# mantasu/face-crop-plus

Measured on AMD Instinct MI355X. Metric: faces/sec end-to-end (detect+align+crop), higher is better.
Workload: dtype f16x3; 1 GPU; RetinaFace detect + 5-pt align/crop, batch=32/GPU synthetic 1024x1024 RGB, strategy=largest, det_threshold=0.6, output 256x256, detector on 2 HIP streams x 16 images; global_batch=32, image_size=1024, parallelism=dp1

## Files before the change

face-crop-plus_amd/csrc/fcp_stem_pool.hip:

```cpp
#include "fcp_conv_common.h"

using namespace fcp_conv;

namespace {

typedef _Float16 f16x2 __attribute__((ext_vector_type(2)));

constexpr int PH = 5;
constexpr int SH = 2 * PH + 1;
constexpr int IH = 2 * SH + 5;
constexpr int SPITCH = 68;
constexpr int KSTEPS = 11;

struct StemGeo {
  static constexpr int PW = 16;
  static constexpr int SW = 2 * PW + 1;
  static constexpr int NSTEM = SH * SW;
  static constexpr int NTILES = (NSTEM + 31) / 32;
  static constexpr int IWB = (2 * SW + 5) * 3;
  static constexpr int IPITCH = 6 * SW + 18;
  static constexpr int IN_ELEMS = (IH + 1) * IPITCH;
  static constexpr int NT = 32 * PW;
  static constexpr int NGRP = NT / 128;
  static constexpr int TPR = NT / 28;
  static constexpr int NLOAD = (IWB + TPR - 1) / TPR;
  static constexpr int C1ROWS = (PH * PW + 31) / 32 * 32;
  static constexpr int C1_BYTES = C1ROWS * 2 * 128;
  static constexpr int WGS = 1;
  static_assert(TPR % 3 == 0 && IH * TPR <= NT && IPITCH % 2 == 0 && NTILES % NGRP == 0, "stem patch geometry");
};

struct StemParams {
  const uint8_t* img;
  const float* imgf;
  const uint32_t* wfrag;
  const float* bias;
  const float* wscale;
  float* out;
  int n, h, w, hs, ws, hp, wp, out_ld, out_fmt;
  int tiles_y, tiles_x, npatches;
  int mean[3];
  const char* w1;
  const float* ws1;
  const float* b1;
  float* t1;
  int t1_ld;
};

constexpr int CPITCH = 68;
__device__ __forceinline__ int swz1(int row) { return ((row >> 1) & 7) ^ ((row & 1) << 2); }

__device__ __forceinline__ void lds_barrier() {
  asm volatile("s_waitcnt lgkmcnt(0)" ::: "memory");
  __builtin_amdgcn_s_barrier();
  asm volatile("" ::: "memory");
}

template <bool HAS_C1, bool F32IN = false>
__global__ void __launch_bounds__(StemGeo::NT, StemGeo::WGS) stem_pool_kernel(const StemParams p) {
  static_assert(!(HAS_C1 && F32IN), "the fp32-input stem has no conv1 tail");
  using G = StemGeo;
  constexpr int PW = G::PW, SW = G::SW, NSTEM = G::NSTEM, NTILES = G::NTILES, IWB = G::IWB, IPITCH = G::IPITCH;
  constexpr int IN_ELEMS = G::IN_ELEMS, NT = G::NT, NGRP = G::NGRP, TPR = G::TPR, NLOAD = G::NLOAD, C1ROWS = G::C1ROWS;
  constexpr int KPG = NTILES / NGRP;
  extern __shared__ __attribute__((aligned(16))) float smem[];
  __shared__ __attribute__((aligned(16))) _Float16 inh[IN_ELEMS];
  __shared__ __attribute__((aligned(16))) _Float16 inl[F32IN ? IN_ELEMS : 8];
  float* stage = smem;
  char* c1in = reinterpret_cast<char*>(smem + NSTEM * SPITCH);

  const int tid = threadIdx.x;
  const int lane = tid & 63;
  const int wave = __builtin_amdgcn_readfirstlane(tid >> 6);
  const int half = lane >> 5;

  const int ct = wave & 1, grp = wave >> 1;
  f16x8 wh[KSTEPS], wl[KSTEPS];
#pragma unroll
  for (int q = 0; q < KSTEPS; ++q) {
    const u32x4_t* src = reinterpret_cast<const u32x4_t*>(p.wfrag) + ((ct * KSTEPS + q) * 2) * 64 + lane;
    wh[q] = __builtin_bit_cast(f16x8, src[0]);
    wl[q] = __builtin_bit_cast(f16x8, src[64]);
  }

  const int pc2 = 2 * (tid & 31), pcol = tid >> 5;
  const float ws2a = p.wscale[pc2], ws2b = p.wscale[pc2 + 1], bias2a = p.bias[pc2], bias2b = p.bias[pc2 + 1];
  float ws1a = 0.f, ws1b = 0.f, b1a = 0.f, b1b = 0.f;
  if constexpr (HAS_C1) { ws1a = p.ws1[pc2]; ws1b = p.ws1[pc2 + 1]; b1a = p.b1[pc2]; b1b = p.b1[pc2 + 1]; }
  const int c1rt = wave >> 1, c1ct = wave & 1;

  const int frow = tid / TPR, fc0 = tid - frow * TPR;
  const int fx0 = fc0 / 3, fch = fc0 - fx0 * 3;
  const int fmean = fch == 0 ? p.mean[0] : (fch == 1 ? p.mean[1] : p.mean[2]);
  _Float16* const fdst = inh + min(frow, IH - 1) * IPITCH + fc0;
  uint8_t pre[F32IN ? 1 : NLOAD];
  float pref[F32IN ? NLOAD : 1];
  unsigned pre_ok = 0u;
  auto fetch = [&](int patch) {
    const int pxi = patch % p.tiles_x;
    const int pyi = (patch / p.tiles_x) % p.tiles_y;
    const int ni = patch / (p.tiles_x * p.tiles_y);
    const int iy0 = 4 * pyi * PH - 5, ix0 = 4 * pxi * PW - 5;
    const int y = iy0 + frow;
    const bool rowok = (unsigned)y < (unsigned)p.h && frow < IH;
    const int yc = min(max(y, 0), p.h - 1);
    const uint8_t* base = p.img + ((long)ni * p.h + yc) * p.w * 3 + fch;
    const float* basef = p.imgf + ((long)ni * p.h + yc) * p.w * 4 + fch;
    pre_ok = 0u;
#pragma unroll
    for (int j = 0; j < NLOAD; ++j) {
      const int x = ix0 + fx0 + (TPR / 3) * j;
      pre_ok |= (rowok && (unsigned)x < (unsigned)p.w) ? (1u << j) : 0u;
      if constexpr (F32IN) pref[j] = basef[(unsigned)(min(max(x, 0), p.w - 1) * 4)];
      else pre[j] = base[(unsigned)(min(max(x, 0), p.w - 1) * 3)];
    }
  };
  _Float16* const fdstl = inl + (F32IN ? min(frow, IH - 1) * IPITCH + fc0 : 0);
  auto commit = [&]() {
    if (frow < IH) {
#pragma unroll
      for (int j = 0; j < NLOAD; ++j) {
        if (fc0 + TPR * j < IWB) {
          if constexpr (F32IN) {
            const float v = ((pre_ok >> j) & 1u) ? pref[j] : 0.f;
            const unsigned hu = __builtin_bit_cast(unsigned, __builtin_amdgcn_cvt_pkrtz(v, 0.f));
            const unsigned lu = __builtin_bit_cast(unsigned, __builtin_amdgcn_cvt_pkrtz(fcp_mix_diff<0>(v, hu), 0.f));
            fdst[TPR * j] = __builtin_bit_cast(_Float16, (unsigned short)(hu & 0xFFFFu));
            fdstl[TPR * j] = __builtin_bit_cast(_Float16, (unsigned short)(lu & 0xFFFFu));
          } else {
            fdst[TPR * j] = (_Float16)(float)(((pre_ok >> j) & 1u) ? (int)pre[j] - fmean : 0);
          }
        }
      }
    }
  };

  for (int i = tid; i < IN_ELEMS / 2; i += NT) {
    reinterpret_cast<uint32_t*>(inh)[i] = 0u;
    if constexpr (F32IN) reinterpret_cast<uint32_t*>(inl)[i] = 0u;
  }
  __syncthreads();

  int abase_t[KPG];
#pragma unroll
  for (int k = 0; k < KPG; ++k) {
    int pix = (grp + NGRP * k) * 32 + (lane & 31);
    pix = pix < NSTEM ? pix : NSTEM - 1;
    const int si = pix / SW, sj = pix - si * SW;
    abase_t[k] = (2 * si) * IPITCH + 6 * sj;
  }

  int patch = blockIdx.x;
  if (patch < p.npatches) fetch(patch);
  for (; patch < p.npatches; patch += gridDim.x) {
    commit();
    lds_barrier();
    const int next = patch + gridDim.x;
    if (next < p.npatches) fetch(next);

    const int pxi = patch % p.tiles_x;
    const int pyi = (patch / p.tiles_x) % p.tiles_y;
    const int ni = patch / (p.tiles_x * p.tiles_y);
    const int py0 = pyi * PH, px0 = pxi * PW;
    const int sy0 = 2 * py0 - 1, sx0 = 2 * px0 - 1;
    const bool interior = sy0 >= 0 && sy0 + SH <= p.hs && sx0 >= 0 && sx0 + SW <= p.ws;

#pragma unroll
    for (int k = 0; k < KPG; ++k) {
      const int t = grp + NGRP * k;
      const int abase = abase_t[k];
      f32x16 acc;
#pragma unroll
      for (int e = 0; e < 16; ++e) acc[e] = 0.f;
      auto afrag_of = [&](const _Float16* plane, int q) {
        const int ch = 2 * q + half;
        const int kh = ch / 3, part = ch - kh * 3;
        const uint32_t* wp = reinterpret_cast<const uint32_t*>(plane + abase + kh * IPITCH + 8 * part);
        const u32x4_t raw = {wp[0], wp[1], wp[2], wp[3]};
        return __builtin_bit_cast(f16x8, raw);
      };
      auto afrag = [&](int q) { return afrag_of(inh, q); };
      f16x8 a = afrag(0), al = a;
      if constexpr (F32IN) al = afrag_of(inl, 0);
#pragma unroll
      for (int q = 0; q < KSTEPS; ++q) {
        f16x8 an = a, aln = al;
        if (q + 1 < KSTEPS) {
          an = afrag(q + 1);
          if constexpr (F32IN) aln = afrag_of(inl, q + 1);
        }
        __builtin_amdgcn_sched_barrier(0);
        if constexpr (F32IN) {
          acc = __builtin_amdgcn_mfma_f32_32x32x16_f16(wh[q], al, acc, 0, 0, 0);
          acc = __builtin_amdgcn_mfma_f32_32x32x16_f16(wl[q], a, acc, 0, 0, 0);
          acc = __builtin_amdgcn_mfma_f32_32x32x16_f16(wh[q], a, acc, 0, 0, 0);
        } else {
          acc = __builtin_amdgcn_mfma_f32_32x32x16_f16(wl[q], a, acc, 0, 0, 0);
          acc = __builtin_amdgcn_mfma_f32_32x32x16_f16(wh[q], a, acc, 0, 0, 0);
        }
        a = an; al = aln;
      }
      {
        const int row = t * 32 + (lane & 31);
        bool in = true;
        if (!interior) {
          const int si = row / SW, sj = row - si * SW;
          in = (unsigned)(sy0 + si) < (unsigned)p.hs && (unsigned)(sx0 + sj) < (unsigned)p.ws;
        }
        if (row < NSTEM) {
          float* dst = stage + row * SPITCH + ct * 32 + 4 * half;
#pragma unroll
          for (int g = 0; g < 4; ++g)
            *reinterpret_cast<f32x4*>(dst + 8 * g) = in ? f32x4{acc[4 * g], acc[4 * g + 1], acc[4 * g + 2], acc[4 * g + 3]}
                                                        : f32x4{-INFINITY, -INFINITY, -INFINITY, -INFINITY};
        }
      }
    }
    lds_barrier();

    f16x8 c1w[8];
    if constexpr (HAS_C1) {
      if (c1rt < C1ROWS / 32) {
        const char* wrow = p.w1 + (size_t)(c1ct * 32 + (lane & 31)) * 256;
#pragma unroll
        for (int sl = 0; sl < 2; ++sl)
#pragma unroll
          for (int sh = 0; sh < 2; ++sh) {
            c1w[(sl * 2 + sh) * 2] = *reinterpret_cast<const f16x8*>(wrow + sl * 128 + (2 * sh + half) * 16);
            c1w[(sl * 2 + sh) * 2 + 1] = *reinterpret_cast<const f16x8*>(wrow + sl * 128 + (4 + 2 * sh + half) * 16);
          }
      }
    }
    {
      typedef float f32x2 __attribute__((ext_vector_type(2)));
      const float* sp = stage + (2 * pcol) * SPITCH + pc2;
      f32x2 rm[SH];
#pragma unroll
      for (int si = 0; si < SH; ++si) {
        const f32x2 a = *reinterpret_cast<const f32x2*>(sp + (si * SW) * SPITCH);
        const f32x2 b = *reinterpret_cast<const f32x2*>(sp + (si * SW + 1) * SPITCH);
        const f32x2 c = *reinterpret_cast<const f32x2*>(sp + (si * SW + 2) * SPITCH);
        rm[si][0] = fmaxf(fmaxf(a[0], b[0]), c[0]);
        rm[si][1] = fmaxf(fmaxf(a[1], b[1]), c[1]);
      }
      const int ox = px0 + pcol;
#pragma unroll
      for (int py = 0; py < PH; ++py) {
        const int oy = py0 + py;
        if (oy >= p.hp || ox >= p.wp) continue;
        float v0 = fmaxf(fmaxf(rm[2 * py][0], rm[2 * py + 1][0]), rm[2 * py + 2][0]) * ws2a + bias2a;
        float v1 = fmaxf(fmaxf(rm[2 * py][1], rm[2 * py + 1][1]), rm[2 * py + 2][1]) * ws2b + bias2b;
        v0 = v0 > 0.f ? v0 : 0.f;
        v1 = v1 > 0.f ? v1 : 0.f;
        const long pixel = ((long)ni * p.hp + oy) * p.wp + ox;
        if (p.out_fmt == 1) {
          unsigned hu, lu;
          split2(v0, v1, hu, lu);
          char* ob = reinterpret_cast<char*>(p.out) + pixel * p.out_ld * 4 + split_chan_off(pc2);
          *reinterpret_cast<unsigned*>(ob) = hu;
          *reinterpret_cast<unsigned*>(ob + 64) = lu;
          if constexpr (HAS_C1) {
            const int pp = py * PW + pcol;
            const int q = (pc2 & 31) >> 3, sw = swz1(pp);
            char* trow = c1in + pp * 256 + (pc2 >> 5) * 128 + (pc2 & 7) * 2;
            *reinterpret_cast<unsigned*>(trow + ((q ^ sw) << 4)) = hu;
            *reinterpret_cast<unsigned*>(trow + (((4 + q) ^ sw) << 4)) = lu;
          }
        } else {
          *reinterpret_cast<f32x2*>(p.out + pixel * p.out_ld + pc2) = f32x2{v0, v1};
        }
      }
    }
    if constexpr (HAS_C1) {
      lds_barrier();
      if (c1rt < C1ROWS / 32) {
        f32x16 acc;
#pragma unroll
        for (int e = 0; e < 16; ++e) acc[e] = 0.f;
        const int row = c1rt * 32 + (lane & 31), sw = swz1(row);
        const char* arow = c1in + row * 256;
#pragma unroll
        for (int sl = 0; sl < 2; ++sl)
#pragma unroll
          for (int sh = 0; sh < 2; ++sh) {
            const f16x8 bh = c1w[(sl * 2 + sh) * 2], bl = c1w[(sl * 2 + sh) * 2 + 1];
            const f16x8 ah = *reinterpret_cast<const f16x8*>(arow + sl * 128 + (((2 * sh + half) ^ sw) << 4));
            const f16x8 al = *reinterpret_cast<const f16x8*>(arow + sl * 128 + (((4 + 2 * sh + half) ^ sw) << 4));
            acc = __builtin_amdgcn_mfma_f32_32x32x16_f16(bh, al, acc, 0, 0, 0);
            acc = __builtin_amdgcn_mfma_f32_32x32x16_f16(bl, ah, acc, 0, 0, 0);
            acc = __builtin_amdgcn_mfma_f32_32x32x16_f16(bh, ah, acc, 0, 0, 0);
          }
        float* dst = stage + row * CPITCH + c1ct * 32 + 4 * half;
#pragma unroll
        for (int g = 0; g < 4; ++g)
          *reinterpret_cast<f32x4*>(dst + 8 * g) = f32x4{acc[4 * g], acc[4 * g + 1], acc[4 * g + 2], acc[4 * g + 3]};
      }
      lds_barrier();
      {
        typedef float f32x2 __attribute__((ext_vector_type(2)));
        const int ox = px0 + pcol;
        f32x2 cv[PH];
#pragma unroll
        for (int py = 0; py < PH; ++py) cv[py] = *reinterpret_cast<const f32x2*>(stage + (py * PW + pcol) * CPITCH + pc2);
#pragma unroll
        for (int py = 0; py < PH; ++py) {
          const int oy = py0 + py;
          if (oy >= p.hp || ox >= p.wp) continue;
          const float x0 = conv_value_relu(cv[py][0], ws1a, b1a), x1 = conv_value_relu(cv[py][1], ws1b, b1b);
          unsigned hu, lu;
          split2(x0, x1, hu, lu);
          const long pixel = ((long)ni * p.hp + oy) * p.wp + ox;
          char* ob = reinterpret_cast<char*>(p.t1) + pixel * p.t1_ld * 4 + split_chan_off(pc2);
          *reinterpret_cast<unsigned*>(ob) = hu;
          *reinterpret_cast<unsigned*>(ob + 64) = lu;
        }
      }
    }
    lds_barrier();
  }
}

}

extern "C" int fcp_stem7x7s2_relu_pool_conv1_u8(const uint8_t* images, int n, int h, int w, const int32_t* mean_rgb,
                                                const void* wfrag, const float* bias, const float* wscale, float* out,
                                                int out_ld, int out_fmt, const void* w1, const float* ws1, const float* b1,
                                                float* t1, int t1_ld, fcp_stream_t stream) {
  FCP_REQUIRE(images && wfrag && bias && wscale && out && mean_rgb, "stem: null pointer");
  const bool has_c1 = w1 != nullptr;
  if (has_c1) {
    FCP_REQUIRE(ws1 && b1 && t1, "stem + conv1: conv1 needs its scales, bias and output");
    FCP_REQUIRE(out_fmt == 1, "stem + conv1: the pooled map must be written in split32 (its bytes are conv1's operand)");
    FCP_REQUIRE(t1_ld >= 64 && t1_ld % 32 == 0 && ((uintptr_t)t1 & 127) == 0 && ((uintptr_t)w1 & 15) == 0,
                "stem + conv1: misaligned conv1 filter / output view");
  }
  FCP_REQUIRE(n > 0 && h >= 1 && w >= 1 && (long)h * w * 3 < (1L << 31), "stem: bad image size");
  FCP_REQUIRE((unsigned)out_fmt <= 1u, "stem: out_fmt must be 0 (fp32) or 1 (split32)");
  FCP_REQUIRE(out_ld >= 64 && out_ld % (out_fmt ? 32 : 4) == 0 && ((uintptr_t)out & (out_fmt ? 127 : 15)) == 0,
              "stem: misaligned output view");
  FCP_REQUIRE(((uintptr_t)wfrag & 15) == 0, "stem: filter fragments must be 16-byte aligned");
  for (int c = 0; c < 3; ++c) FCP_REQUIRE(mean_rgb[c] >= 0 && mean_rgb[c] <= 255, "stem: means must be integers in 0..255");
  StemParams p = {};
  p.img = images; p.wfrag = static_cast<const uint32_t*>(wfrag); p.bias = bias; p.wscale = wscale; p.out = out;
  p.n = n; p.h = h; p.w = w;
  p.hs = (h + 6 - 7) / 2 + 1; p.ws = (w + 6 - 7) / 2 + 1;
  p.hp = (p.hs + 2 - 3) / 2 + 1; p.wp = (p.ws + 2 - 3) / 2 + 1;
  p.out_ld = out_ld; p.out_fmt = out_fmt;
  p.tiles_y = fcp_cdiv(p.hp, PH); p.tiles_x = fcp_cdiv(p.wp, StemGeo::PW);
  const long np = (long)n * p.tiles_y * p.tiles_x;
  FCP_REQUIRE(np < (1L << 31) && (long)n * h * w * 3 < (1L << 40), "stem: batch too large");
  p.npatches = (int)np;
  for (int c = 0; c < 3; ++c) p.mean[c] = mean_rgb[c];
  p.w1 = static_cast<const char*>(w1); p.ws1 = ws1; p.b1 = b1; p.t1 = t1; p.t1_ld = t1_ld;
  using G = StemGeo;
  const size_t lds = (size_t)G::NSTEM * SPITCH * 4 + (has_c1 ? G::C1_BYTES : 0);
  const int cus = fcp_cu_count() * G::WGS;
  const int grid = (int)(np < cus ? np : cus);
  if (has_c1) {
    FCP_LDS_OPT_IN((&stem_pool_kernel<true>), lds);
    hipLaunchKernelGGL((stem_pool_kernel<true>), dim3(grid), dim3(G::NT), lds, (hipStream_t)stream, p);
  } else {
    FCP_LDS_OPT_IN((&stem_pool_kernel<false>), lds);
    hipLaunchKernelGGL((stem_pool_kernel<false>), dim3(grid), dim3(G::NT), lds, (hipStream_t)stream, p);
  }
  FCP_LAUNCH_OK();
  return 0;
}

extern "C" int fcp_stem7x7s2_relu_pool_f32(const float* x4, int n, int h, int w, const void* wfrag, const float* bias,
                                           const float* wscale, float* out, int out_ld, int out_fmt, fcp_stream_t stream) {
  FCP_REQUIRE(x4 && wfrag && bias && wscale && out, "stem(f32): null pointer");
  FCP_REQUIRE(n > 0 && h >= 1 && w >= 1 && (long)h * w * 4 < (1L << 31), "stem(f32): bad image size");
  FCP_REQUIRE((unsigned)out_fmt <= 1u, "stem(f32): out_fmt must be 0 (fp32) or 1 (split32)");
  FCP_REQUIRE(out_ld >= 64 && out_ld % (out_fmt ? 32 : 4) == 0 && ((uintptr_t)out & (out_fmt ? 127 : 15)) == 0,
              "stem(f32): misaligned output view");
  FCP_REQUIRE(((uintptr_t)wfrag & 15) == 0 && ((uintptr_t)x4 & 15) == 0, "stem(f32): input / filter fragments must be 16-byte aligned");
  using G = StemGeo;
  StemParams p = {};
  p.imgf = x4; p.wfrag = static_cast<const uint32_t*>(wfrag); p.bias = bias; p.wscale = wscale; p.out = out;
  p.n = n; p.h = h; p.w = w;
  p.hs = (h + 6 - 7) / 2 + 1; p.ws = (w + 6 - 7) / 2 + 1;
  p.hp = (p.hs + 2 - 3) / 2 + 1; p.wp = (p.ws + 2 - 3) / 2 + 1;
  p.out_ld = out_ld; p.out_fmt = out_fmt;
  p.tiles_y = fcp_cdiv(p.hp, PH); p.tiles_x = fcp_cdiv(p.wp, G::PW);
  const long np = (long)n * p.tiles_y * p.tiles_x;
  FCP_REQUIRE(np < (1L << 31) && (long)n * h * w * 4 < (1L << 40), "stem(f32): batch too large");
  p.npatches = (int)np;
  const size_t lds = (size_t)G::NSTEM * SPITCH * 4;
  const int cus = fcp_cu_count() * G::WGS;
  const int grid = (int)(np < cus ? np : cus);
  FCP_LDS_OPT_IN((&stem_pool_kernel<false, true>), lds);
  hipLaunchKernelGGL((stem_pool_kernel<false, true>), dim3(grid), dim3(G::NT), lds, (hipStream_t)stream, p);
  FCP_LAUNCH_OK();
  return 0;
}

extern "C" int fcp_stem7x7s2_relu_pool_u8(const uint8_t* images, int n, int h, int w, const int32_t* mean_rgb,
                                          const void* wfrag, const float* bias, const float* wscale, float* out,
                                          int out_ld, int out_fmt, fcp_stream_t stream) {
  return fcp_stem7x7s2_relu_pool_conv1_u8(images, n, h, w, mean_rgb, wfrag, bias, wscale, out, out_ld, out_fmt, nullptr, nullptr,
                                          nullptr, nullptr, 0, stream);
}
```

Before: 1457 faces/s.

## Warp-specialize stem kernel into MFMA and load/pool waves with double-buffered input

Splits the stem workgroup into matrix waves, which run the 7x7 conv MFMAs and the conv1 tail, and service waves, which fetch the next patch into a double-buffered LDS input tile and do the 3x3 max-pool plus output. The stem tiles are computed in two strips so pooling of the first strip overlaps conv of the second. Conv1 filters are preloaded into registers once, and conv1 for the previous patch is interleaved into the next round, writing the output straight from MFMA accumulators instead of restaging it through LDS. This is meant to hide global loads and pooling behind tensor work. In exchange it adds LDS, register pressure and fragile barrier choreography, and halves the threads doing loads.

```diff
diff --git a/face-crop-plus_amd/csrc/fcp_stem_pool.hip b/face-crop-plus_amd/csrc/fcp_stem_pool.hip
--- a/face-crop-plus_amd/csrc/fcp_stem_pool.hip
+++ b/face-crop-plus_amd/csrc/fcp_stem_pool.hip
@@ -5,6 +5,8 @@
 namespace {
 
 typedef _Float16 f16x2 __attribute__((ext_vector_type(2)));
+typedef float f32x2 __attribute__((ext_vector_type(2)));
+typedef unsigned int u32x2_t __attribute__((ext_vector_type(2)));
 
 constexpr int PH = 5;
 constexpr int SH = 2 * PH + 1;
@@ -21,13 +23,20 @@
   static constexpr int IPITCH = 6 * SW + 18;
   static constexpr int IN_ELEMS = (IH + 1) * IPITCH;
   static constexpr int NT = 32 * PW;
-  static constexpr int NGRP = NT / 128;
-  static constexpr int TPR = NT / 28;
+  static constexpr int NSVC = NT / 2;
+  static constexpr int NGRP = 2;
+  static constexpr int KPG = NTILES / NGRP;
+  static constexpr int SROW = PH;
+  static constexpr int STAGE_PIX = NSTEM + SW;
+  static constexpr int TPR = NSVC / 28;
   static constexpr int NLOAD = (IWB + TPR - 1) / TPR;
   static constexpr int C1ROWS = (PH * PW + 31) / 32 * 32;
   static constexpr int C1_BYTES = C1ROWS * 2 * 128;
   static constexpr int WGS = 1;
-  static_assert(TPR % 3 == 0 && IH * TPR <= NT && IPITCH % 2 == 0 && NTILES % NGRP == 0, "stem patch geometry");
+  static_assert(TPR % 3 == 0 && IH * TPR <= NSVC && IPITCH % 2 == 0 && NTILES % (2 * NGRP) == 0 && NLOAD <= 32, "stem patch geometry");
+  static_assert(NTILES / 2 * 32 >= SROW * SW && NTILES / 2 * 32 < (SROW + 1) * SW && SROW % 2 == 1, "strip boundary");
+  static_assert(C1ROWS == 96 && (SROW / 2) * PW == 32, "conv1 row tile 0 = the pooled rows of the first strip");
+  static constexpr size_t lds_bytes(bool has_c1) { return (size_t)STAGE_PIX * SPITCH * 4 + (has_c1 ? C1_BYTES : 0); }
 };
 
 struct StemParams {
@@ -47,7 +56,6 @@
   int t1_ld;
 };
 
-constexpr int CPITCH = 68;
 __device__ __forceinline__ int swz1(int row) { return ((row >> 1) & 7) ^ ((row & 1) << 2); }
 
 __device__ __forceinline__ void lds_barrier() {
@@ -56,56 +64,86 @@
   asm volatile("" ::: "memory");
 }
 
+struct PatchAt {
+  int ni, py0, px0, sy0, sx0;
+};
+
 template <bool HAS_C1, bool F32IN = false>
 __global__ void __launch_bounds__(StemGeo::NT, StemGeo::WGS) stem_pool_kernel(const StemParams p) {
   static_assert(!(HAS_C1 && F32IN), "the fp32-input stem has no conv1 tail");
   using G = StemGeo;
-  constexpr int PW = G::PW, SW = G::SW, NSTEM = G::NSTEM, NTILES = G::NTILES, IWB = G::IWB, IPITCH = G::IPITCH;
-  constexpr int IN_ELEMS = G::IN_ELEMS, NT = G::NT, NGRP = G::NGRP, TPR = G::TPR, NLOAD = G::NLOAD, C1ROWS = G::C1ROWS;
-  constexpr int KPG = NTILES / NGRP;
+  constexpr int PW = G::PW, SW = G::SW, NSTEM = G::NSTEM, IWB = G::IWB, IPITCH = G::IPITCH, SROW = G::SROW;
+  constexpr int IN_ELEMS = G::IN_ELEMS, NT = G::NT, NGRP = G::NGRP, TPR = G::TPR, NLOAD = G::NLOAD, KPG = G::KPG;
   extern __shared__ __attribute__((aligned(16))) float smem[];
-  __shared__ __attribute__((aligned(16))) _Float16 inh[IN_ELEMS];
-  __shared__ __attribute__((aligned(16))) _Float16 inl[F32IN ? IN_ELEMS : 8];
+  __shared__ __attribute__((aligned(16))) _Float16 inh[2 * IN_ELEMS];
+  __shared__ __attribute__((aligned(16))) _Float16 inl[F32IN ? 2 * IN_ELEMS : 8];
   float* stage = smem;
-  char* c1in = reinterpret_cast<char*>(smem + NSTEM * SPITCH);
+  char* c1in = reinterpret_cast<char*>(smem + G::STAGE_PIX * SPITCH);
 
   const int tid = threadIdx.x;
   const int lane = tid & 63;
   const int wave = __builtin_amdgcn_readfirstlane(tid >> 6);
   const int half = lane >> 5;
-
-  const int ct = wave & 1, grp = wave >> 1;
+  const bool matrix = wave < NT / 128;
+
+  const int ct = wave & 1, grp = (wave >> 1) & 1;
   f16x8 wh[KSTEPS], wl[KSTEPS];
-#pragma unroll
-  for (int q = 0; q < KSTEPS; ++q) {
-    const u32x4_t* src = reinterpret_cast<const u32x4_t*>(p.wfrag) + ((ct * KSTEPS + q) * 2) * 64 + lane;
-    wh[q] = __builtin_bit_cast(f16x8, src[0]);
-    wl[q] = __builtin_bit_cast(f16x8, src[64]);
-  }
-
-  const int pc2 = 2 * (tid & 31), pcol = tid >> 5;
+  f16x8 c1w[HAS_C1 ? 8 : 1];
+  f32x4 c1s[HAS_C1 ? 4 : 1], c1b[HAS_C1 ? 4 : 1];
+  auto load_filters = [&]() {
+#pragma unroll
+    for (int q = 0; q < KSTEPS; ++q) {
+      const u32x4_t* src = reinterpret_cast<const u32x4_t*>(p.wfrag) + ((ct * KSTEPS + q) * 2) * 64 + lane;
+      wh[q] = __builtin_bit_cast(f16x8, src[0]);
+      wl[q] = __builtin_bit_cast(f16x8, src[64]);
+    }
+    if constexpr (HAS_C1) {
+      const char* wrow = p.w1 + (size_t)(ct * 32 + (lane & 31)) * 256;
+#pragma unroll
+      for (int sl = 0; sl < 2; ++sl)
+#pragma unroll
+        for (int sh = 0; sh < 2; ++sh) {
+          c1w[(sl * 2 + sh) * 2] = *reinterpret_cast<const f16x8*>(wrow + sl * 128 + (2 * sh + half) * 16);
+          c1w[(sl * 2 + sh) * 2 + 1] = *reinterpret_cast<const f16x8*>(wrow + sl * 128 + (4 + 2 * sh + half) * 16);
+        }
+#pragma unroll
+      for (int g = 0; g < 4; ++g)
+#pragma unroll
+        for (int e = 0; e < 4; ++e) {
+          c1s[g][e] = p.ws1[ct * 32 + 8 * g + 4 * half + e];
+          c1b[g][e] = p.b1[ct * 32 + 8 * g + 4 * half + e];
+        }
+    }
+  };
+
+  const int stid = tid & (G::NSVC - 1);
+  const int pc2 = 2 * (stid & 31), pcol0 = stid >> 5;
   const float ws2a = p.wscale[pc2], ws2b = p.wscale[pc2 + 1], bias2a = p.bias[pc2], bias2b = p.bias[pc2 + 1];
-  float ws1a = 0.f, ws1b = 0.f, b1a = 0.f, b1b = 0.f;
-  if constexpr (HAS_C1) { ws1a = p.ws1[pc2]; ws1b = p.ws1[pc2 + 1]; b1a = p.b1[pc2]; b1b = p.b1[pc2 + 1]; }
-  const int c1rt = wave >> 1, c1ct = wave & 1;
-
-  const int frow = tid / TPR, fc0 = tid - frow * TPR;
+
+  const int frow = stid / TPR, fc0 = stid % TPR;
   const int fx0 = fc0 / 3, fch = fc0 - fx0 * 3;
   const int fmean = fch == 0 ? p.mean[0] : (fch == 1 ? p.mean[1] : p.mean[2]);
-  _Float16* const fdst = inh + min(frow, IH - 1) * IPITCH + fc0;
+  const int foff = min(frow, IH - 1) * IPITCH + fc0;
   uint8_t pre[F32IN ? 1 : NLOAD];
   float pref[F32IN ? NLOAD : 1];
   unsigned pre_ok = 0u;
-  auto fetch = [&](int patch) {
+  auto patch_at = [&](int patch) {
     const int pxi = patch % p.tiles_x;
     const int pyi = (patch / p.tiles_x) % p.tiles_y;
-    const int ni = patch / (p.tiles_x * p.tiles_y);
-    const int iy0 = 4 * pyi * PH - 5, ix0 = 4 * pxi * PW - 5;
+    PatchAt a;
+    a.ni = patch / (p.tiles_x * p.tiles_y);
+    a.py0 = pyi * PH; a.px0 = pxi * PW;
+    a.sy0 = 2 * a.py0 - 1; a.sx0 = 2 * a.px0 - 1;
+    return a;
+  };
+  auto fetch = [&](int patch) {
+    const PatchAt a = patch_at(patch);
+    const int iy0 = 4 * a.py0 - 5, ix0 = 4 * a.px0 - 5;
     const int y = iy0 + frow;
     const bool rowok = (unsigned)y < (unsigned)p.h && frow < IH;
     const int yc = min(max(y, 0), p.h - 1);
-    const uint8_t* base = p.img + ((long)ni * p.h + yc) * p.w * 3 + fch;
-    const float* basef = p.imgf + ((long)ni * p.h + yc) * p.w * 4 + fch;
+    const uint8_t* base = p.img + ((long)a.ni * p.h + yc) * p.w * 3 + fch;
+    const float* basef = p.imgf + ((long)a.ni * p.h + yc) * p.w * 4 + fch;
     pre_ok = 0u;
 #pragma unroll
     for (int j = 0; j < NLOAD; ++j) {
@@ -115,9 +153,10 @@
       else pre[j] = base[(unsigned)(min(max(x, 0), p.w - 1) * 3)];
     }
   };
-  _Float16* const fdstl = inl + (F32IN ? min(frow, IH - 1) * IPITCH + fc0 : 0);
-  auto commit = [&]() {
+  auto commit = [&](int buf) {
     if (frow < IH) {
+      _Float16* const fdst = inh + buf * IN_ELEMS + foff;
+      _Float16* const fdstl = inl + (F32IN ? buf * IN_ELEMS + foff : 0);
 #pragma unroll
       for (int j = 0; j < NLOAD; ++j) {
         if (fc0 + TPR * j < IWB) {
@@ -135,188 +174,233 @@
     }
   };
 
-  for (int i = tid; i < IN_ELEMS / 2; i += NT) {
+  for (int i = tid; i < IN_ELEMS; i += NT) {
     reinterpret_cast<uint32_t*>(inh)[i] = 0u;
     if constexpr (F32IN) reinterpret_cast<uint32_t*>(inl)[i] = 0u;
   }
   __syncthreads();
 
-  int abase_t[KPG];
+  int abase_t[KPG], soff_t[KPG];
+  unsigned srow = 0u;
 #pragma unroll
   for (int k = 0; k < KPG; ++k) {
-    int pix = (grp + NGRP * k) * 32 + (lane & 31);
-    pix = pix < NSTEM ? pix : NSTEM - 1;
+    const int px = (grp + NGRP * k) * 32 + (lane & 31);
+    const int pix = px < NSTEM ? px : NSTEM - 1;
     const int si = pix / SW, sj = pix - si * SW;
     abase_t[k] = (2 * si) * IPITCH + 6 * sj;
+    soff_t[k] = px * SPITCH + ct * 32 + 4 * half;
+    srow |= si == SROW ? (1u << k) : 0u;
   }
 
-  int patch = blockIdx.x;
-  if (patch < p.npatches) fetch(patch);
-  for (; patch < p.npatches; patch += gridDim.x) {
-    commit();
-    lds_barrier();
-    const int next = patch + gridDim.x;
-    if (next < p.npatches) fetch(next);
-
-    const int pxi = patch % p.tiles_x;
-    const int pyi = (patch / p.tiles_x) % p.tiles_y;
-    const int ni = patch / (p.tiles_x * p.tiles_y);
-    const int py0 = pyi * PH, px0 = pxi * PW;
-    const int sy0 = 2 * py0 - 1, sx0 = 2 * px0 - 1;
-    const bool interior = sy0 >= 0 && sy0 + SH <= p.hs && sx0 >= 0 && sx0 + SW <= p.ws;
-
-#pragma unroll
-    for (int k = 0; k < KPG; ++k) {
-      const int t = grp + NGRP * k;
-      const int abase = abase_t[k];
-      f32x16 acc;
-#pragma unroll
-      for (int e = 0; e < 16; ++e) acc[e] = 0.f;
-      auto afrag_of = [&](const _Float16* plane, int q) {
-        const int ch = 2 * q + half;
-        const int kh = ch / 3, part = ch - kh * 3;
-        const uint32_t* wp = reinterpret_cast<const uint32_t*>(plane + abase + kh * IPITCH + 8 * part);
-        const u32x4_t raw = {wp[0], wp[1], wp[2], wp[3]};
-        return __builtin_bit_cast(f16x8, raw);
-      };
-      auto afrag = [&](int q) { return afrag_of(inh, q); };
-      f16x8 a = afrag(0), al = a;
-      if constexpr (F32IN) al = afrag_of(inl, 0);
-#pragma unroll
-      for (int q = 0; q < KSTEPS; ++q) {
-        f16x8 an = a, aln = al;
-        if (q + 1 < KSTEPS) {
-          an = afrag(q + 1);
-          if constexpr (F32IN) aln = afrag_of(inl, q + 1);
-        }
-        __builtin_amdgcn_sched_barrier(0);
-        if constexpr (F32IN) {
-          acc = __builtin_amdgcn_mfma_f32_32x32x16_f16(wh[q], al, acc, 0, 0, 0);
-          acc = __builtin_amdgcn_mfma_f32_32x32x16_f16(wl[q], a, acc, 0, 0, 0);
-          acc = __builtin_amdgcn_mfma_f32_32x32x16_f16(wh[q], a, acc, 0, 0, 0);
-        } else {
-          acc = __builtin_amdgcn_mfma_f32_32x32x16_f16(wl[q], a, acc, 0, 0, 0);
-          acc = __builtin_amdgcn_mfma_f32_32x32x16_f16(wh[q], a, acc, 0, 0, 0);
-        }
-        a = an; al = aln;
-      }
-      {
-        const int row = t * 32 + (lane & 31);
-        bool in = true;
-        if (!interior) {
-          const int si = row / SW, sj = row - si * SW;
-          in = (unsigned)(sy0 + si) < (unsigned)p.hs && (unsigned)(sx0 + sj) < (unsigned)p.ws;
-        }
-        if (row < NSTEM) {
-          float* dst = stage + row * SPITCH + ct * 32 + 4 * half;
-#pragma unroll
-          for (int g = 0; g < 4; ++g)
-            *reinterpret_cast<f32x4*>(dst + 8 * g) = in ? f32x4{acc[4 * g], acc[4 * g + 1], acc[4 * g + 2], acc[4 * g + 3]}
-                                                        : f32x4{-INFINITY, -INFINITY, -INFINITY, -INFINITY};
-        }
-      }
-    }
-    lds_barrier();
-
-    f16x8 c1w[8];
-    if constexpr (HAS_C1) {
-      if (c1rt < C1ROWS / 32) {
-        const char* wrow = p.w1 + (size_t)(c1ct * 32 + (lane & 31)) * 256;
-#pragma unroll
-        for (int sl = 0; sl < 2; ++sl)
-#pragma unroll
-          for (int sh = 0; sh < 2; ++sh) {
-            c1w[(sl * 2 + sh) * 2] = *reinterpret_cast<const f16x8*>(wrow + sl * 128 + (2 * sh + half) * 16);
-            c1w[(sl * 2 + sh) * 2 + 1] = *reinterpret_cast<const f16x8*>(wrow + sl * 128 + (4 + 2 * sh + half) * 16);
-          }
-      }
-    }
-    {
-      typedef float f32x2 __attribute__((ext_vector_type(2)));
+  auto afrag_of = [&](const _Float16* plane, int k, int buf, int q) {
+    const int ch = 2 * q + half;
+    const int kh = ch / 3, part = ch - kh * 3;
+    const uint32_t* wp = reinterpret_cast<const uint32_t*>(plane + abase_t[k] + buf * IN_ELEMS + kh * IPITCH + 8 * part);
+    const u32x4_t raw = {wp[0], wp[1], wp[2], wp[3]};
+    return __builtin_bit_cast(f16x8, raw);
+  };
+  f16x8 a, al;
+  auto first_frag = [&](int k, int buf) {
+    a = afrag_of(inh, k, buf, 0);
+    al = a;
+    if constexpr (F32IN) al = afrag_of(inl, k, buf, 0);
+  };
+  auto stem_tile = [&](int k, bool NEXT, const PatchAt& at, int buf, bool interior) {
+    const int t = grp + NGRP * k;
+    f32x16 acc;
+#pragma unroll
+    for (int e = 0; e < 16; ++e) acc[e] = 0.f;
+#pragma unroll
+    for (int q = 0; q < KSTEPS; ++q) {
+      f16x8 an = a, aln = al;
+      if (q + 1 < KSTEPS || NEXT) {
+        const int kn = q + 1 < KSTEPS ? k : k + 1, qn = q + 1 < KSTEPS ? q + 1 : 0;
+        an = afrag_of(inh, kn, buf, qn);
+        if constexpr (F32IN) aln = afrag_of(inl, kn, buf, qn);
+      }
+      __builtin_amdgcn_sched_barrier(0);
+      if constexpr (F32IN) {
+        acc = __builtin_amdgcn_mfma_f32_32x32x16_f16(wh[q], al, acc, 0, 0, 0);
+        acc = __builtin_amdgcn_mfma_f32_32x32x16_f16(wl[q], a, acc, 0, 0, 0);
+        acc = __builtin_amdgcn_mfma_f32_32x32x16_f16(wh[q], a, acc, 0, 0, 0);
+      } else {
+        acc = __builtin_amdgcn_mfma_f32_32x32x16_f16(wl[q], a, acc, 0, 0, 0);
+        acc = __builtin_amdgcn_mfma_f32_32x32x16_f16(wh[q], a, acc, 0, 0, 0);
+      }
+      a = an; al = aln;
+    }
+    const int row = t * 32 + (lane & 31);
+    bool in = true;
+    if (!interior) {
+      const int si = row / SW, sj = row - si * SW;
+      in = (unsigned)(at.sy0 + si) < (unsigned)p.hs && (unsigned)(at.sx0 + sj) < (unsigned)p.ws;
+    }
+    if (row < NSTEM) {
+      float* dst = stage + soff_t[k] + (((srow >> k) & 1u) && buf ? (NSTEM - SROW * SW) * SPITCH : 0);
+#pragma unroll
+      for (int g = 0; g < 4; ++g)
+        *reinterpret_cast<f32x4*>(dst + 8 * g) = in ? f32x4{acc[4 * g], acc[4 * g + 1], acc[4 * g + 2], acc[4 * g + 3]}
+                                                    : f32x4{-INFINITY, -INFINITY, -INFINITY, -INFINITY};
+    }
+  };
+
+  auto emit = [&](const PatchAt& at, int py, int pcol, float m0, float m1) {
+    const int oy = at.py0 + py, ox = at.px0 + pcol;
+    if (oy >= p.hp || ox >= p.wp) return;
+    float v0 = m0 * ws2a + bias2a;
+    float v1 = m1 * ws2b + bias2b;
+    v0 = v0 > 0.f ? v0 : 0.f;
+    v1 = v1 > 0.f ? v1 : 0.f;
+    const long pixel = ((long)at.ni * p.hp + oy) * p.wp + ox;
+    if (p.out_fmt == 1) {
+      unsigned hu, lu;
+      split2(v0, v1, hu, lu);
+      char* ob = reinterpret_cast<char*>(p.out) + pixel * p.out_ld * 4 + split_chan_off(pc2);
+      *reinterpret_cast<unsigned*>(ob) = hu;
+      *reinterpret_cast<unsigned*>(ob + 64) = lu;
+      if constexpr (HAS_C1) {
+        const int pp = py * PW + pcol;
+        const int q = (pc2 & 31) >> 3, sw = swz1(pp);
+        char* trow = c1in + pp * 256 + (pc2 >> 5) * 128 + (pc2 & 7) * 2;
+        *reinterpret_cast<unsigned*>(trow + ((q ^ sw) << 4)) = hu;
+        *reinterpret_cast<unsigned*>(trow + (((4 + q) ^ sw) << 4)) = lu;
+      }
+    } else {
+      *reinterpret_cast<f32x2*>(p.out + pixel * p.out_ld + pc2) = f32x2{v0, v1};
+    }
+  };
+  f32x2 carry[2];
+  auto hmax = [&](const float* rowp) {
+    const f32x2 a = *reinterpret_cast<const f32x2*>(rowp);
+    const f32x2 b = *reinterpret_cast<const f32x2*>(rowp + SPITCH);
+    const f32x2 c = *reinterpret_cast<const f32x2*>(rowp + 2 * SPITCH);
+    return f32x2{fmaxf(fmaxf(a[0], b[0]), c[0]), fmaxf(fmaxf(a[1], b[1]), c[1])};
+  };
+  auto pool_first = [&](const PatchAt& at) {
+#pragma unroll
+    for (int j = 0; j < 2; ++j) {
+      const int pcol = pcol0 + (PW / 2) * j;
+      const float* sp = stage + (2 * pcol) * SPITCH + pc2;
+      f32x2 rm[SROW];
+#pragma unroll
+      for (int si = 0; si < SROW; ++si) rm[si] = hmax(sp + (si * SW) * SPITCH);
+#pragma unroll
+      for (int py = 0; py < SROW / 2; ++py)
+        emit(at, py, pcol, fmaxf(fmaxf(rm[2 * py][0], rm[2 * py + 1][0]), rm[2 * py + 2][0]),
+             fmaxf(fmaxf(rm[2 * py][1], rm[2 * py + 1][1]), rm[2 * py + 2][1]));
+      carry[j] = rm[SROW - 1];
+    }
+  };
+  auto pool_second = [&](const PatchAt& at, int buf) {
+#pragma unroll
+    for (int j = 0; j < 2; ++j) {
+      const int pcol = pcol0 + (PW / 2) * j;
       const float* sp = stage + (2 * pcol) * SPITCH + pc2;
       f32x2 rm[SH];
-#pragma unroll
-      for (int si = 0; si < SH; ++si) {
-        const f32x2 a = *reinterpret_cast<const f32x2*>(sp + (si * SW) * SPITCH);
-        const f32x2 b = *reinterpret_cast<const f32x2*>(sp + (si * SW + 1) * SPITCH);
-        const f32x2 c = *reinterpret_cast<const f32x2*>(sp + (si * SW + 2) * SPITCH);
-        rm[si][0] = fmaxf(fmaxf(a[0], b[0]), c[0]);
-        rm[si][1] = fmaxf(fmaxf(a[1], b[1]), c[1]);
-      }
-      const int ox = px0 + pcol;
-#pragma unroll
-      for (int py = 0; py < PH; ++py) {
-        const int oy = py0 + py;
-        if (oy >= p.hp || ox >= p.wp) continue;
-        float v0 = fmaxf(fmaxf(rm[2 * py][0], rm[2 * py + 1][0]), rm[2 * py + 2][0]) * ws2a + bias2a;
-        float v1 = fmaxf(fmaxf(rm[2 * py][1], rm[2 * py + 1][1]), rm[2 * py + 2][1]) * ws2b + bias2b;
-        v0 = v0 > 0.f ? v0 : 0.f;
-        v1 = v1 > 0.f ? v1 : 0.f;
-        const long pixel = ((long)ni * p.hp + oy) * p.wp + ox;
-        if (p.out_fmt == 1) {
-          unsigned hu, lu;
-          split2(v0, v1, hu, lu);
-          char* ob = reinterpret_cast<char*>(p.out) + pixel * p.out_ld * 4 + split_chan_off(pc2);
-          *reinterpret_cast<unsigned*>(ob) = hu;
-          *reinterpret_cast<unsigned*>(ob + 64) = lu;
-          if constexpr (HAS_C1) {
-            const int pp = py * PW + pcol;
-            const int q = (pc2 & 31) >> 3, sw = swz1(pp);
-            char* trow = c1in + pp * 256 + (pc2 >> 5) * 128 + (pc2 & 7) * 2;
-            *reinterpret_cast<unsigned*>(trow + ((q ^ sw) << 4)) = hu;
-            *reinterpret_cast<unsigned*>(trow + (((4 + q) ^ sw) << 4)) = lu;
-          }
-        } else {
-          *reinterpret_cast<f32x2*>(p.out + pixel * p.out_ld + pc2) = f32x2{v0, v1};
-        }
-      }
-    }
-    if constexpr (HAS_C1) {
+      rm[SROW - 1] = carry[j];
+      rm[SROW] = hmax(sp + (buf ? NSTEM : SROW * SW) * SPITCH);
+#pragma unroll
+      for (int si = SROW + 1; si < SH; ++si) rm[si] = hmax(sp + (si * SW) * SPITCH);
+#pragma unroll
+      for (int py = SROW / 2; py < PH; ++py)
+        emit(at, py, pcol, fmaxf(fmaxf(rm[2 * py][0], rm[2 * py + 1][0]), rm[2 * py + 2][0]),
+             fmaxf(fmaxf(rm[2 * py][1], rm[2 * py + 1][1]), rm[2 * py + 2][1]));
+    }
+  };
+
+  auto conv1_tile = [&](int rt, const PatchAt& at) {
+    f32x16 acc;
+#pragma unroll
+    for (int e = 0; e < 16; ++e) acc[e] = 0.f;
+    const int pp = rt * 32 + (lane & 31), sw = swz1(pp);
+    const char* arow = c1in + pp * 256;
+#pragma unroll
+    for (int sl = 0; sl < 2; ++sl)
+#pragma unroll
+      for (int sh = 0; sh < 2; ++sh) {
+        const f16x8 bh = c1w[(sl * 2 + sh) * 2], bl = c1w[(sl * 2 + sh) * 2 + 1];
+        const f16x8 ah = *reinterpret_cast<const f16x8*>(arow + sl * 128 + (((2 * sh + half) ^ sw) << 4));
+        const f16x8 al = *reinterpret_cast<const f16x8*>(arow + sl * 128 + (((4 + 2 * sh + half) ^ sw) << 4));
+        acc = __builtin_amdgcn_mfma_f32_32x32x16_f16(bh, al, acc, 0, 0, 0);
+        acc = __builtin_amdgcn_mfma_f32_32x32x16_f16(bl, ah, acc, 0, 0, 0);
+        acc = __builtin_amdgcn_mfma_f32_32x32x16_f16(bh, ah, acc, 0, 0, 0);
+      }
+    const int py = pp / PW, pcol = pp - py * PW;
+    const int oy = at.py0 + py, ox = at.px0 + pcol;
+    if (py >= PH || oy >= p.hp || ox >= p.wp) return;
+    const long pixel = ((long)at.ni * p.hp + oy) * p.wp + ox;
+    char* ob = reinterpret_cast<char*>(p.t1) + pixel * p.t1_ld * 4 + split_chan_off(ct * 32 + 4 * half);
+#pragma unroll
+    for (int g = 0; g < 4; ++g) {
+      unsigned hu0, lu0, hu1, lu1;
+      split2(conv_value_relu(acc[4 * g], c1s[g][0], c1b[g][0]), conv_value_relu(acc[4 * g + 1], c1s[g][1], c1b[g][1]), hu0, lu0);
+      split2(conv_value_relu(acc[4 * g + 2], c1s[g][2], c1b[g][2]), conv_value_relu(acc[4 * g + 3], c1s[g][3], c1b[g][3]), hu1, lu1);
+      *reinterpret_cast<u32x2_t*>(ob + 16 * g) = u32x2_t{hu0, hu1};
+      *reinterpret_cast<u32x2_t*>(ob + 16 * g + 64) = u32x2_t{lu0, lu1};
+    }
+  };
+
+  struct Round {
+    bool have, have_next;
+    int next, buf;
+    PatchAt at;
+  };
+  auto round_of = [&](int i, int patch) {
+    Round r;
+    r.have = patch < p.npatches;
+    r.next = patch + gridDim.x;
+    r.have_next = r.have && r.next < p.npatches;
+    r.buf = i & 1;
+    r.at = patch_at(r.have ? patch : 0);
+    return r;
+  };
+  int patch = blockIdx.x;
+  PatchAt prev = {};
+  if (matrix) {
+    load_filters();
+    lds_barrier();
+    for (int i = 0;; ++i) {
+      const Round r = round_of(i, patch);
+      const PatchAt& at = r.at;
+      const bool interior = at.sy0 >= 0 && at.sy0 + SH <= p.hs && at.sx0 >= 0 && at.sx0 + SW <= p.ws;
+      if (r.have) {
+        first_frag(0, r.buf);
+#pragma unroll
+        for (int k = 0; k < KPG / 2; ++k) stem_tile(k, k + 1 < KPG / 2, at, r.buf, interior);
+      }
+      if constexpr (HAS_C1) {
+        if (i > 0 && wave < 2) conv1_tile(0, prev);
+      }
       lds_barrier();
-      if (c1rt < C1ROWS / 32) {
-        f32x16 acc;
-#pragma unroll
-        for (int e = 0; e < 16; ++e) acc[e] = 0.f;
-        const int row = c1rt * 32 + (lane & 31), sw = swz1(row);
-        const char* arow = c1in + row * 256;
-#pragma unroll
-        for (int sl = 0; sl < 2; ++sl)
-#pragma unroll
-          for (int sh = 0; sh < 2; ++sh) {
-            const f16x8 bh = c1w[(sl * 2 + sh) * 2], bl = c1w[(sl * 2 + sh) * 2 + 1];
-            const f16x8 ah = *reinterpret_cast<const f16x8*>(arow + sl * 128 + (((2 * sh + half) ^ sw) << 4));
-            const f16x8 al = *reinterpret_cast<const f16x8*>(arow + sl * 128 + (((4 + 2 * sh + half) ^ sw) << 4));
-            acc = __builtin_amdgcn_mfma_f32_32x32x16_f16(bh, al, acc, 0, 0, 0);
-            acc = __builtin_amdgcn_mfma_f32_32x32x16_f16(bl, ah, acc, 0, 0, 0);
-            acc = __builtin_amdgcn_mfma_f32_32x32x16_f16(bh, ah, acc, 0, 0, 0);
-          }
-        float* dst = stage + row * CPITCH + c1ct * 32 + 4 * half;
-#pragma unroll
-        for (int g = 0; g < 4; ++g)
-          *reinterpret_cast<f32x4*>(dst + 8 * g) = f32x4{acc[4 * g], acc[4 * g + 1], acc[4 * g + 2], acc[4 * g + 3]};
-      }
+      if (r.have) {
+        first_frag(KPG / 2, r.buf);
+#pragma unroll
+        for (int k = KPG / 2; k < KPG; ++k) stem_tile(k, k + 1 < KPG, at, r.buf, interior);
+      }
+      if constexpr (HAS_C1) {
+        if (i > 0) conv1_tile(1 + (wave >> 1), prev);
+      }
+      if (!r.have) break;
       lds_barrier();
-      {
-        typedef float f32x2 __attribute__((ext_vector_type(2)));
-        const int ox = px0 + pcol;
-        f32x2 cv[PH];
-#pragma unroll
-        for (int py = 0; py < PH; ++py) cv[py] = *reinterpret_cast<const f32x2*>(stage + (py * PW + pcol) * CPITCH + pc2);
-#pragma unroll
-        for (int py = 0; py < PH; ++py) {
-          const int oy = py0 + py;
-          if (oy >= p.hp || ox >= p.wp) continue;
-          const float x0 = conv_value_relu(cv[py][0], ws1a, b1a), x1 = conv_value_relu(cv[py][1], ws1b, b1b);
-          unsigned hu, lu;
-          split2(x0, x1, hu, lu);
-          const long pixel = ((long)ni * p.hp + oy) * p.wp + ox;
-          char* ob = reinterpret_cast<char*>(p.t1) + pixel * p.t1_ld * 4 + split_chan_off(pc2);
-          *reinterpret_cast<unsigned*>(ob) = hu;
-          *reinterpret_cast<unsigned*>(ob + 64) = lu;
-        }
-      }
-    }
+      prev = at;
+      patch = r.next;
+    }
+  } else {
+    fetch(patch);
+    commit(0);
     lds_barrier();
+    for (int i = 0;; ++i) {
+      const Round r = round_of(i, patch);
+      if (r.have_next) fetch(r.next);
+      if (i > 0) pool_second(prev, r.buf ^ 1);
+      lds_barrier();
+      if (!r.have) break;
+      pool_first(r.at);
+      if (r.have_next) commit(r.buf ^ 1);
+      lds_barrier();
+      prev = r.at;
+      patch = r.next;
+    }
   }
 }
 
@@ -353,7 +437,7 @@
   for (int c = 0; c < 3; ++c) p.mean[c] = mean_rgb[c];
   p.w1 = static_cast<const char*>(w1); p.ws1 = ws1; p.b1 = b1; p.t1 = t1; p.t1_ld = t1_ld;
   using G = StemGeo;
-  const size_t lds = (size_t)G::NSTEM * SPITCH * 4 + (has_c1 ? G::C1_BYTES : 0);
+  const size_t lds = G::lds_bytes(has_c1);
   const int cus = fcp_cu_count() * G::WGS;
   const int grid = (int)(np < cus ? np : cus);
   if (has_c1) {
@@ -386,7 +470,7 @@
   const long np = (long)n * p.tiles_y * p.tiles_x;
   FCP_REQUIRE(np < (1L << 31) && (long)n * h * w * 4 < (1L << 40), "stem(f32): batch too large");
   p.npatches = (int)np;
-  const size_t lds = (size_t)G::NSTEM * SPITCH * 4;
+  const size_t lds = G::lds_bytes(false);
   const int cus = fcp_cu_count() * G::WGS;
   const int grid = (int)(np < cus ? np : cus);
   FCP_LDS_OPT_IN((&stem_pool_kernel<false, true>), lds);
```

Measured after the change: 1471 faces/s, median of 6. No clear change (+0.9%).
